# lmmontoya-ai/taboo-brittleness

Measured on AMD Instinct MI355X. Metric: prompts/sec SAE-ablation sweep Gemma-2-9B @L32, higher is better.
Workload: dtype bf16

## Files before the change

taboo_brittleness_amd/csrc/api.h:

```cpp
#pragma once
#include <hip/hip_runtime.h>
#include <stdint.h>

void tb_rmsnorm(const uint16_t* x, const uint16_t* w, uint16_t* y, int M, int D, float eps, hipStream_t st);
void tb_add_rmsnorm2(uint16_t* h, const uint16_t* o, const uint16_t* w_post, const uint16_t* w_next, uint16_t* x,
                     int M, int D, float eps, hipStream_t st);
void tb_embed_rmsnorm(const int32_t* ids, const uint16_t* E, const uint16_t* w, uint16_t* h, uint16_t* x, int M,
                      int D, int V, float scale, float eps, hipStream_t st);
void tb_rope_qkv_cache(const uint16_t* qkv, const int32_t* pos, const int32_t* slot_of_row, const float* cos_t,
                       const float* sin_t, uint16_t* q_out, uint16_t* kc, uint16_t* vc, int M, int Hq, int Hkv,
                       int HD, int S, int max_pos, hipStream_t st);
void tb_rope_qkv_cache_part(const float* part, int ks, const int32_t* pos, const int32_t* slot_of_row,
                            const float* cos_t, const float* sin_t, uint16_t* q_out, uint16_t* kc, uint16_t* vc, int M,
                            int Hq, int Hkv, int HD, int S, int max_pos, hipStream_t st);
void tb_kv_fanout(uint16_t* kc, uint16_t* vc, const int32_t* src_row, const int32_t* slot, const int32_t* pos, int M,
                  int nlayers, int slots, int Hkv, int S, int HD, hipStream_t st);
int tb_attention_lds_bytes(int HD);
int tb_attention_split_rows(int n, bool prefix);
void tb_attention(const uint16_t* q, const uint16_t* kc, const uint16_t* vc, uint16_t* out, const int32_t* pos,
                  const int32_t* slot, int B, int T, int Hq, int Hkv, int HD, int S, float scale, float softcap,
                  int window, hipStream_t st, const uint16_t* pkc = nullptr, const uint16_t* pvc = nullptr,
                  const int32_t* pslot = nullptr, const int32_t* plen = nullptr);
void tb_attention_varlen(const uint16_t* q, const uint16_t* kc, const uint16_t* vc, uint16_t* out, const int32_t* pos,
                         const int32_t* blk, int nblk, int Hq, int Hkv, int HD, int S, float scale, float softcap,
// ... 35 lines not shown
bool tb_gemm4_ok(int M, int N, int K);
int tb_gemm4_set_pipe(int on);
int tb_gemm4_splitk_ks(int M, int N, int K, int tile_rows);
int tb_gemm4_splitk_part(const uint16_t* A, const uint16_t* W, float* ws, int M, int N, int K, int tile_rows, int ks,
                         hipStream_t st);
void tb_add_rmsnorm2_part(uint16_t* h, const float* part, int ks, const uint16_t* w_post, const uint16_t* w_next,
                          uint16_t* x, int M, int D, float eps, hipStream_t st);
void tb_gemm4_splitk(const uint16_t* A, const uint16_t* W, uint16_t* out, float* ws, int M, int N, int K, int ldo,
                     int epi, int tile_rows, int ks, hipStream_t st);
void tb_row_combine(const int64_t* ptr, const float* coef, float* out, int B, int T, int V, hipStream_t st);
bool tb_random_basis_ok(int D);
void tb_random_basis(const uint64_t* seeds, const int32_t* ranks, const int64_t* rows, int n, int D, float* table,
                     hipStream_t st, int qu = 1);
void tb_gemm4(const uint16_t* A, const uint16_t* W, void* C, const float* bias, const float* thr, int M, int N, int K,
              int ldc, int epi, int tile_rows, hipStream_t st, const uint16_t* a2 = nullptr, int k0 = 0);
void tb_gemm_nt(const uint16_t* A, const uint16_t* W, void* C, const float* bias, const float* thr, int M, int N,
                int K, int ldc, int epi, hipStream_t st);
void tb_lowrank_edit(uint16_t* h, uint16_t* x_next, const uint8_t* apply, const int32_t* idx, const int32_t* cnt,
                     int mmax, const void* E, const void* Dm, int table_f32, const float* bias, const float* thr,
                     const float* pre_bias, float alpha, const uint16_t* w_next, float eps, int M, int D,
                     float* coef_out, hipStream_t st, const float* val = nullptr);
void tb_interchange_edit(uint16_t* h, uint16_t* x_next, const uint8_t* apply, const int32_t* idx, const int32_t* cnt,
                         int mmax, const void* E, const void* Dm, int table_f32, const float* bias, const float* thr,
                         const float* pre_bias, float alpha, const uint16_t* w_next, float eps, int M, int D,
                         float* coef_out, const uint16_t* donor, const int32_t* src, int n_donor, float* dcoef_out,
                         hipStream_t st);
void tb_matched_noise_edit(uint16_t* h, uint16_t* x_next, const uint8_t* apply, const int32_t* idx,
                           const int32_t* cnt, int mmax, const void* E, const void* Dm, int table_f32,
                           const float* bias, const float* thr, const float* pre_bias, float alpha,
                           const uint16_t* w_next, float eps, int M, int D, float* coef_out, const float* val,
// ... 68 lines not shown
```

taboo_brittleness_amd/csrc/bindings.cpp:

```cpp
#include <torch/extension.h>
#include <ATen/hip/impl/HIPStreamMasqueradingAsCUDA.h>
#include <c10/core/DeviceGuard.h>

#include <cstdlib>

#include "api.h"

namespace {

hipStream_t cur_stream() { return c10::hip::getCurrentHIPStreamMasqueradingAsCUDA().stream(); }

#define CHECK_DEV(t) TORCH_CHECK((t).is_cuda(), #t " must be a GPU tensor")
#define CHECK_CONTIG(t) TORCH_CHECK((t).is_contiguous(), #t " must be contiguous")
#define CHECK_BF16(t) TORCH_CHECK((t).scalar_type() == at::kBFloat16, #t " must be bfloat16")
#define CHECK_F32(t) TORCH_CHECK((t).scalar_type() == at::kFloat, #t " must be float32")
#define CHECK_I32(t) TORCH_CHECK((t).scalar_type() == at::kInt, #t " must be int32")
#define CHECK_U8(t) TORCH_CHECK((t).scalar_type() == at::kByte || (t).scalar_type() == at::kBool, #t " must be uint8/bool")
#define IN_BF16(t) CHECK_DEV(t); CHECK_CONTIG(t); CHECK_BF16(t)
#define IN_F32(t) CHECK_DEV(t); CHECK_CONTIG(t); CHECK_F32(t)
#define IN_I32(t) CHECK_DEV(t); CHECK_CONTIG(t); CHECK_I32(t)
#define IN_U8(t) CHECK_DEV(t); CHECK_CONTIG(t); CHECK_U8(t)

bool debug_checks() {
  static const bool on = [] {
// ... 589 lines not shown
void gemm4_qkv_rope(torch::Tensor x, torch::Tensor w, torch::Tensor pos, torch::Tensor slot_of_row, torch::Tensor cs,
                    torch::Tensor q_out, torch::Tensor kc, torch::Tensor vc, int64_t Hq, int64_t Hkv,
                    int64_t tile_rows, OptTensor a2) {
  IN_BF16(x); IN_BF16(w);
  int K = x.size(-1), M = pos.numel(), k0 = 0;
  if (given(a2)) l2a_check(x, *a2, w, M, K, k0);
  TORCH_CHECK(x.numel() == (int64_t)M * (k0 ? k0 : K), "gemm4_qkv_rope: x must be [M, K] with M = pos.numel()");
  qkv_l2a_check(pos, slot_of_row, cs, q_out, kc, vc, M, Hq, Hkv, w);
  TORCH_CHECK(w.size(1) == K, "gemm4_qkv_rope: K mismatch");
  TORCH_CHECK(tb_gemm4_ok(M, w.size(0), K), "gemm4_qkv_rope: need K % 64 == 0, K >= 64");
  TORCH_CHECK(tile_rows == 256 || tile_rows == 128, "gemm4_qkv_rope: tile_rows must be 256 or 128");
  c10::DeviceGuard g(x.device());
  tb_gemm4_qkv_rope(cbf(x), cbf(w), pos.data_ptr<int32_t>(), slot_of_row.data_ptr<int32_t>(), cbf(cs),
                    bf(q_out), bf(kc), bf(vc), M, K, Hq, Hkv, kc.size(2), cs.size(0),
                    (int)tile_rows, cur_stream(), k0 ? cbf(*a2) : nullptr, k0);
}

void row_combine(torch::Tensor ptr, torch::Tensor coef, torch::Tensor out) {
  CHECK_DEV(ptr); CHECK_CONTIG(ptr); IN_F32(coef); IN_F32(out);
  TORCH_CHECK(ptr.scalar_type() == at::kLong && ptr.dim() == 2 && coef.sizes() == ptr.sizes(),
              "row_combine: ptr int64 [B, T], coef f32 [B, T]");
  const int B = ptr.size(0), T = ptr.size(1), V = out.size(-1);
  TORCH_CHECK(out.numel() == (int64_t)B * V && V % 4 == 0, "row_combine: out [B, V], V % 4 == 0");
  c10::DeviceGuard g(out.device());
  tb_row_combine(ptr.data_ptr<int64_t>(), coef.data_ptr<float>(), out.data_ptr<float>(), B, T, V, cur_stream());
}

void random_basis(torch::Tensor seeds, torch::Tensor ranks, torch::Tensor rows, torch::Tensor table, int64_t qu) {
  CHECK_DEV(seeds); CHECK_CONTIG(seeds); CHECK_DEV(ranks); CHECK_CONTIG(ranks); CHECK_DEV(rows); CHECK_CONTIG(rows);
  IN_F32(table);
// ... 605 lines not shown
  m.def("gemm_nt", &gemm_nt);
  m.def("gemm4", &gemm4, "A"_a, "W"_a, "C"_a, "bias"_a, "thr"_a, "epi"_a, "tile_rows"_a, a2);
  m.def("gemm4_ok", &gemm4_ok);
  m.def("gemm4_set_pipe", &gemm4_set_pipe);
  m.def("gemm_ring", &gemm_ring, "A"_a, "W"_a, "C"_a, "epi"_a, "bm"_a, "bn"_a, "var"_a, a2);
  m.def("gemm_ring_ok", &gemm_ring_ok);
  m.def("gemm_ring_tiles", &gemm_ring_tiles);
  m.def("gemm_ring_qkv_rope", &gemm_ring_qkv_rope, "x"_a, "w"_a, "pos"_a, "slot_of_row"_a, "cs"_a, "q_out"_a,
        "kc"_a, "vc"_a, "Hq"_a, "Hkv"_a, "bm"_a, "bn"_a, "var"_a, a2);
  m.def("gemm4_splitk", &gemm4_splitk);
  m.def("gemm4_splitk_ks", &gemm4_splitk_ks);
  m.def("gemm4_splitk_part", &gemm4_splitk_part);
  m.def("add_rmsnorm2_part", &add_rmsnorm2_part);
  m.def("gemm4_qkv_rope", &gemm4_qkv_rope, "x"_a, "w"_a, "pos"_a, "slot_of_row"_a, "cs"_a, "q_out"_a, "kc"_a,
        "vc"_a, "Hq"_a, "Hkv"_a, "tile_rows"_a, a2);
  m.def("lora_t", &lora_t);
  m.def("lora_t_chunks", &lora_t_chunks);
  m.def("row_combine", &row_combine);
  m.def("random_basis", &random_basis);
  m.def("lora_t_ok", &lora_t_ok);
  m.def("head_fused", &head_fused);
  m.def("lens_gemm", &lens_gemm);
  m.def("lowrank_edit", &lowrank_edit);
  m.def("latent_affine_edit", &latent_affine_edit);
  m.def("matched_noise_edit", &matched_noise_edit);
  m.def("interchange_edit", &interchange_edit);
  m.def("sae_decode_sparse", &sae_decode_sparse);
  m.def("sae_splice_edit", &sae_splice_edit);
  m.def("flag_compact", &flag_compact);
  m.def("latent_score", &latent_score);
// ... 19 lines not shown
```

taboo_brittleness_amd/csrc/gemm4.hip:

```cpp
#include "common.h"
#include "api.h"
#include <algorithm>
#include <cstdlib>
#include <utility>

namespace {

constexpr int G4_THREADS = 256, G4_BN = 256;
constexpr int G4_GROUP_M = 4;
constexpr int G4_SLACK1 = 4;
constexpr int G4_SLACK2 = 0;
#ifndef G4_CNT
#define G4_CNT 1
#endif

typedef __attribute__((address_space(3))) void g4_lds_t;
typedef uint32_t u32x2 __attribute__((ext_vector_type(2)));
typedef __attribute__((address_space(3))) char g4_lds_char;

template <int N>
__device__ __forceinline__ void g4_vmcnt() {
  static_assert(N >= 0 && N < 64, "vmcnt range");
  asm volatile("s_waitcnt vmcnt(%0)" ::"n"(N) : "memory");
}
// ... 50 lines not shown
  uint16_t* kc;
  uint16_t* vc;
  int Hq, Hkv, S, max_pos;
  const uint16_t* ctab;
  int clo, chi;
  float csat, crc, ccap;
  const int32_t* tgt;
  float* tgt_logit;
  float* part;
  int ksplit, kchunk;
  const uint16_t* a2;
  int k0;
};
constexpr int G4_CTAB_N = 32768;

template <int BM, int EPI, bool L2A = false, bool PIPE = false>
__global__ void __launch_bounds__(G4_THREADS, 1)
gemm4_kernel(const uint16_t* __restrict__ A, const uint16_t* __restrict__ W, void* __restrict__ C,
             const float* __restrict__ bias, const float* __restrict__ thr, int M, int N, int K, int ldc, G4Rope rp) {
#if defined(__HIP_DEVICE_COMPILE__)
  static_assert(BM == 256 || BM == 128 || (BM == 64 && EPI == G4_F32), "tile rows (64: the split-K decode tile)");
  static_assert(!PIPE || (BM == 256 && !L2A && (EPI == G4_BF16 || EPI == G4_LENS || EPI == G4_GEGLU || EPI == G4_ROPE)),
                "cross-tile stream: 256-row tile, one A source, no split-K");
  static_assert(!PIPE || BM == G4_BN, "PIPE stages A with W's row offsets");
  constexpr bool G4C = G4_CNT && BM == 256;
  constexpr int WN = 8, WM = BM / 32;
  constexpr int PIMG = G4_BN * 128, QIMG = BM * 128, STG = PIMG + QIMG;
  constexpr int PI = G4_BN / 32, QI = BM / 32, GL = PI + QI;
  constexpr bool LEPI = EPI == G4_BF16 || EPI == G4_LENS;
  constexpr int RB = EPI == G4_GEGLU ? 128 : 256, ECH = RB / 16, ERPI = 64 / ECH;
  constexpr bool SPARE = LEPI;
  constexpr int EXB = SPARE ? 32768 : 0;
  constexpr int ERR = SPARE ? EXB / (4 * RB) : EPI == G4_GEGLU ? BM / 2 : BM / 4;
  constexpr int ENR = LEPI ? (BM / 2) / ERPI : 1;
  constexpr int CTB = EPI == G4_HEAD ? 4096 : 0;
  static_assert(2 * STG + CTB + EXB <= 160 * 1024, "LDS");
  __shared__ __attribute__((aligned(1024))) char smem[2 * STG + CTB + EXB];

  const int nbn = N / G4_BN, nbm = (M + BM - 1) / BM, nwg = nbn * nbm;
  const int NT = K >> 6, KS = EPI == G4_F32 && rp.ksplit > 1 ? rp.ksplit : 1, KC = KS > 1 ? rp.kchunk : NT;
  const int nwgv = nwg * KS;
#define G4_TILE(v, m0_, n0_)                                                                              \
  do {                                                                                                    \
    const int q_ = nwgv / 8, r_ = nwgv % 8, x_ = (v) % 8;                                                 \
    int b_ = (x_ < r_ ? x_ * (q_ + 1) : r_ * (q_ + 1) + (x_ - r_) * q_) + (v) / 8;                        \
    sk = b_ / nwg;                                                                                        \
    b_ -= sk * nwg;                                                                                       \
    const int pg_ = G4_GROUP_M * nbn, fb_ = (b_ / pg_) * G4_GROUP_M;                                      \
    const int gs_ = min(nbm - fb_, G4_GROUP_M), l_ = b_ % pg_;                                            \
    m0_ = (fb_ + l_ % gs_) * BM;                                                                          \
    n0_ = (l_ / gs_) * G4_BN;                                                                             \
  } while (0)
  int tile = blockIdx.x, m0, n0, sk;
  G4_TILE(tile, m0, n0);

  const int tid = threadIdx.x, lane = tid & 63;
  const int wid = __builtin_amdgcn_readfirstlane(tid >> 6);
  const int wn = wid & 1, wm = wid >> 1;

  const int lchunk = (lane & 7) ^ ((4 * wid + (lane >> 4)) & 7);
  const int wbytes = G4_BN * K * 2;
  const int KA = L2A ? rp.k0 : K, K2 = K - KA, NT0 = KA >> 6;
  uint32_t vp[PI], vq[QI], vq2[L2A ? QI : 1];
#pragma unroll
  for (int i = 0; i < PI; ++i) vp[i] = (uint32_t)((8 * (4 * i + wid) + (lane >> 3)) * K + lchunk * 8) * 2u;
  int mrows, abytes, abytes2 = 0, nt;
  void *wtile, *atile, *atile2 = nullptr;
#define G4_DESC()                                                                                 \
  do {                                                                                            \
    mrows = min(BM, M - m0);                                                                      \
    wtile = (void*)(W + (size_t)n0 * K + sk * KC * 64);                                           \
    atile = (void*)(A + (size_t)m0 * KA + sk * KC * 64);                                          \
    nt = min(KC, NT - sk * KC);                                                                   \
    abytes = mrows * KA * 2;                                                                      \
    int ln_ = __builtin_amdgcn_mbcnt_hi(~0u, __builtin_amdgcn_mbcnt_lo(~0u, 0u));    \
    asm volatile("" : "+v"(ln_));                                                                 \
    const int lc_ = (ln_ & 7) ^ ((4 * wid + (ln_ >> 4)) & 7);                                     \
    _Pragma("unroll") for (int i = 0; i < QI; ++i)                                                \
      vq[i] = (uint32_t)(min(8 * (4 * i + wid) + (ln_ >> 3), mrows - 1) * KA + lc_ * 8) * 2u;     \
    if constexpr (L2A) {                                                                          \
      atile2 = (void*)(rp.a2 + (size_t)m0 * K2);                                                  \
      abytes2 = mrows * K2 * 2;                                                                   \
      _Pragma("unroll") for (int i = 0; i < QI; ++i)                                              \
        vq2[L2A ? i : 0] = (uint32_t)(min(8 * (4 * i + wid) + (ln_ >> 3), mrows - 1) * K2 + lc_ * 8) * 2u; \
    }                                                                                             \
  } while (0)
  G4_DESC();
  int par = 0, m0n = 0, n0n = 0, abytes_n = 0;
// ... 98 lines not shown
  const uint32_t bq0 = lds0 + offq - PIMG + co0, bq1 = lds0 + offq - PIMG + co1;

  if constexpr (EPI == G4_HEAD) {
    if (rp.ctab != nullptr) {
      uint16_t* lt = reinterpret_cast<uint16_t*>(smem + 2 * STG);
      for (int i = tid; i < rp.chi - rp.clo; i += G4_THREADS) lt[i] = rp.ctab[i];
    }
    __syncthreads();
  }
  G4_STAGE(0, 0);
  G4_STAGE(min(1, nt - 1), 1);
  if constexpr (PIPE) G4_NEXT();
  bool first_tile = true;
  for (;;) {
  constexpr bool REREAD = PIPE && EPI == G4_ROPE;
  if (!PIPE || first_tile || REREAD) {
  if (!PIPE || first_tile) {
    if (first_tile || !LEPI) g4_vmcnt<GL>();
    else g4_vmcnt<GL + ENR>();
    g4_bar();
  }
  if (G4C) {
    asm volatile("s_waitcnt lgkmcnt(0)" ::: "memory");
    const uint32_t o_ = par * STG;
    g4_rd(p0[0], bp0 + o_, G4_PK(0));
#pragma unroll
    for (int j = 0; j < WM; ++j) g4_rd(q0[j], bq0 + o_, G4_QK(j));
#pragma unroll
    for (int i = 1; i < WN; ++i) g4_rd(p0[i], bp0 + o_, G4_PK(i));
    if constexpr (PIPE) G4_HOLD_FRAGS();
  } else {
#pragma unroll
    for (int i = 0; i < WN; ++i) p0[i] = frag(par, offp + G4_PROW(i) * 128 + co0);
#pragma unroll
// ... 64 lines not shown
    G4_PERIOD(nt - 1, kt1, true, true, false);
  }
#undef G4_PERIOD
  if (G4C) asm volatile("s_waitcnt lgkmcnt(0)" ::: "memory");
#undef G4_WAIT
#undef G4_POST
#undef G4_MF
#undef G4_MFMA
#undef G4_MFMA0
  if constexpr (!PIPE) {
    g4_vmcnt<0>();
    g4_bar();
  } else if (G4C && !REREAD) {
    G4_HOLD_FRAGS();
  }
  const int em0 = m0, en0 = n0, esk = sk;
  const int next = PIPE ? nwgv : tile + (int)gridDim.x;
  const bool more = PIPE ? has_next : next < nwgv;
  if constexpr (PIPE) {
    tile += (int)gridDim.x;
    m0 = m0n;
    n0 = n0n;
    wtile = wtile_n;
    atile = atile_n;
    abytes = abytes_n;
    par ^= nt & 1;
  }
  if constexpr (LEPI) {
    if (next < nwgv) {
      tile = next;
      G4_TILE(tile, m0, n0);
      G4_DESC();
      G4_STAGE(0, 0);
      if constexpr (SPARE) G4_STAGE(min(1, nt - 1), 1);
    }
    asm volatile("s_nop 15\n\ts_nop 15" ::: "memory");
    const uint32_t reg = (uint32_t)(uintptr_t)((g4_lds_char*)smem) + (SPARE ? 2 * STG + CTB : STG) + wid * ERR * RB;
    uint16_t* obase = reinterpret_cast<uint16_t*>(C) + (size_t)(em0 + wm * (BM / 2)) * ldc;
    const int nrow = min(BM / 2, M - em0 - wm * (BM / 2));
    const auto ors = __builtin_amdgcn_make_buffer_rsrc(obase, 0, nrow > 0 ? nrow * ldc * 2 : 0, 0x00020000);
    int ln = __builtin_amdgcn_mbcnt_hi(~0u, __builtin_amdgcn_mbcnt_lo(~0u, 0u));
    asm volatile("" : "+v"(ln));
    const int oc0 = (EPI == G4_GEGLU ? (en0 >> 1) + wn * 64 : en0 + wn * 128) + (ln % ECH) * 8;
    constexpr int NI = EPI == G4_GEGLU ? WN / 2 : WN, NRA = ECH / ERPI;
    uint32_t wa[NI], ra[NRA];
#pragma unroll
    for (int i = 0; i < NI; ++i) {
// ... 26 lines not shown
          g4_ds_write_b64<jj * 16 * RB>(wa[i], w);
        }
      });
      u32x4 ev[ERR / ERPI];
      g4_unroll<ERR / ERPI>([&](auto kc) {
        constexpr int k = decltype(kc)::value;
        g4_ds_read_b128<(k / NRA) * NRA * ERPI * RB>(ev[k], ra[k % NRA]);
      });
      asm volatile("s_waitcnt lgkmcnt(0)" ::: "memory");
#pragma unroll
      for (int k = 0; k < ERR / ERPI; ++k)
        __builtin_amdgcn_raw_buffer_store_b128(ev[k], ors, ((rnd * ERR + ERPI * k + ln / ECH) * ldc + oc0) * 2, 0, 0);
    });
    if constexpr (!SPARE) {
      g4_bar();
      if (next < nwgv) G4_STAGE(min(1, nt - 1), 1);
    }
  }
  int tj[EPI == G4_HEAD ? WM : 1];
  if constexpr (EPI == G4_HEAD) {
#pragma unroll
    for (int j = 0; j < WM; ++j) {
      const int m = em0 + wm * (BM / 2) + (lane & 15) + j * 16;
      tj[j] = -1;
      if (rp.tgt != nullptr) {
        const int t = rp.tgt[min(m, M - 1)];
        tj[j] = m < M ? t : -1;
      }
    }
  }
  constexpr int RWM = EPI == G4_ROPE ? WM : 1, RWN = EPI == G4_ROPE ? WN / 2 : 1;
// ... 4 lines not shown
    const int mb_ = em0 + wm * (BM / 2) + (lane & 15);
#pragma unroll
    for (int j = 0; j < WM; ++j) {
      const int m = min(mb_ + j * 16, M - 1);
      rpos[j] = mb_ + j * 16 < M ? rp.pos[m] : -1;
      rslt[j] = rp.slot[m];
    }
#pragma unroll
    for (int j = 0; j < RPF; ++j) {
      const int pp = min(max(rpos[j], 0), rp.max_pos - 1);
#pragma unroll
      for (int i = 0; i < WN / 2; ++i)
        rcs[j][i] = *reinterpret_cast<const uint4*>(rp.cs + ((size_t)pp * 128 + wn * 64 + i * 16 + 4 * (lane >> 4)) * 2);
    }
  }
  if (!LEPI && next < nwgv) {
    tile = next;
    G4_TILE(tile, m0, n0);
    G4_DESC();
    G4_STAGE(0, 0);
    G4_STAGE(min(1, nt - 1), 1);
  }
  const uint16_t* ct = reinterpret_cast<const uint16_t*>(smem + 2 * STG);
  if constexpr (!LEPI) asm volatile("s_nop 15\n\ts_nop 15" ::: "memory");

  {
  const int nb = en0 + wn * 128 + 4 * (lane >> 4);
  const int mb = em0 + wm * (BM / 2) + (lane & 15);
  if constexpr (EPI == G4_HEAD || EPI == G4_LENS) {
    float4* part = reinterpret_cast<float4*>(EPI == G4_LENS ? rp.part : reinterpret_cast<float*>(C));
    const int npart = N / 128, pcol = (en0 >> 7) + wn;
    const uint32_t ctb = (uint32_t)(uintptr_t)((g4_lds_char*)smem) + 2 * STG;
    constexpr float L2E = 1.4426950408889634f;
#pragma unroll
// ... 158 lines not shown
  } else {
#pragma unroll
    for (int i = 0; i < WN; ++i)
#pragma unroll
      for (int j = 0; j < WM; ++j) acc[i][j] = (f32x4){0.f, 0.f, 0.f, 0.f};
  }
  }
  g4_vmcnt<0>();
#undef G4_STAGE
#undef G4_STAGE_ONE
#undef G4_HOLD_FRAGS
#undef G4_STAGE_PIPE
#undef G4_NEXT
#undef G4_TILE
#undef G4_DESC
#endif
}

template <int EPI>
__global__ void __launch_bounds__(256) g4_splitk_reduce_kernel(const float* __restrict__ part, uint16_t* __restrict__ out,
                                                               int M, int N, int ks, int ldo) {
  const int nout = EPI == G4_GEGLU ? N / 2 : N;
  const size_t i = (size_t)blockIdx.x * blockDim.x + threadIdx.x;
  const int per_row = nout / 8;
  if (i >= (size_t)M * per_row) return;
  const int m = (int)(i / per_row), c8 = (int)(i % per_row) * 8;
  const size_t plane = (size_t)M * N;
  float o[8];
  if constexpr (EPI == G4_GEGLU) {
    const int blk = c8 >> 6, fi = c8 & 63;
// ... 177 lines not shown
  G4Rope rp{pos, slot_of_row, cs, q_out, kc, vc, Hq, Hkv, S, max_pos};
  if (a2 != nullptr) {
    rp.a2 = a2;
    rp.k0 = k0;
    if (tile_rows == 128) G4_GO2(128, G4_ROPE);
    else G4_GO2(256, G4_ROPE);
    return;
  }
  if (tile_rows == 128) G4_GO(128, G4_ROPE);
  else G4_GOP(G4_ROPE);
#undef G4_GOP
#undef G4_GO
#undef G4_GO2
}

namespace {

__global__ void __launch_bounds__(256) head_merge_kernel(const float4* __restrict__ part, int npart,
                                                         const int32_t* __restrict__ tgt,
                                                         const float* __restrict__ tgt_logit, int32_t* __restrict__ nxt,
                                                         float* __restrict__ nll_self, float* __restrict__ nll_tgt,
                                                         float* __restrict__ lse_out, int V) {
  __shared__ float sm[4], ss[4];
  __shared__ int si[4];
  const int r = blockIdx.x;
  const float4* p = part + (size_t)r * npart;
  float mx = -INFINITY, s = 0.f;
  int bi = 0x7fffffff;
  auto merge = [&](float m2, float s2, int i2) {
    if (m2 > mx) { s = (mx == -INFINITY ? 0.f : s * __expf(mx - m2)) + s2; mx = m2; bi = i2; }
// ... 39 lines not shown
```

taboo_brittleness_amd/isa_check.py:

```python
from __future__ import annotations

import os
import re
import subprocess
import sys
import tempfile
from typing import Dict, List, Set, Tuple

CSRC = os.path.join(os.path.dirname(os.path.abspath(__file__)), "csrc")
HIPCC = os.path.join(os.environ.get("ROCM_PATH", "/opt/rocm"), "bin", "hipcc")

_REG = re.compile(r"\b([va])(?:\[(\d+):(\d+)\]|(\d+)(?!\w))")


def _regs(text: str) -> Set[Tuple[str, int]]:
    out = set()
    for m in _REG.finditer(text):
        kind = m.group(1)
        if m.group(4) is not None:
            out.add((kind, int(m.group(4))))
        else:
            out.update((kind, r) for r in range(int(m.group(2)), int(m.group(3)) + 1))
    return out

# ... 49 lines not shown


def loops(asm: str, variants: bool = False) -> Dict[str, Tuple[List[str], List[str]]]:
    funcs: Dict[str, List[str]] = {}
    cur = None
    for line in asm.split("\n"):
        m = re.match(r"^(_Z\S+):", line)
        if m:
            cur = m.group(1)
            funcs[cur] = []
            continue
        if cur is not None:
            funcs[cur].append(line)
    out = {}
    for name, body in funcs.items():
        m = re.search(r"gemm4_kernelILi(\d+)ELi(\d+)E(?:Lb([01])ELb([01])E)?", name)
        if not m or m.group(1) != "256":
            continue
        blocks, cur_b, labels = [], [], [""]
        for line in body:
            if re.match(r"^\.LBB", line):
                blocks.append(cur_b)
                cur_b = []
                labels.append(line.split(":")[0])
            else:
                s = line.strip()
                if s and not s.startswith((";", ".")):
                    cur_b.append(s.split(";")[0].strip())
        blocks.append(cur_b)
        nmf = [sum("mfma" in x for x in b) for b in blocks]
        pipe = m.group(4) == "1"
        if pipe:
# ... 2 lines not shown
            ti = next((i for i in range(li + 1, len(blocks)) if nmf[i] >= 200), None)
        else:
            li = max(range(len(blocks)), key=lambda i: nmf[i])
            ti = li + 1 if li + 1 < len(blocks) else None
        def _top(blk):
            fm = next((i for i, x in enumerate(blk) if "mfma" in x), len(blk))
            nrd = sum(x.startswith("ds_read_b128") for x in blk[:fm])
            return nrd > 0 and (fm == len(blk) or (pipe and nrd >= 16))

        pi = li - 1
        while pi >= 0 and not _top(blocks[pi]):
            pi -= 1
        pre = [x for b in blocks[max(pi, 0): li] for x in b] if pi >= 0 else []
        key = f"gemm4_kernel<256, {m.group(2)}>"
        if variants:
            key = f"gemm4_kernel<256, {m.group(2)}, {m.group(3) or 0}, {m.group(4) or 0}>"
        elif key in out and (pipe or m.group(3) == "1"):
            continue
        out[key] = (pre, blocks[li])
        tail = []
        if ti is not None:
            last = max([i for i, x in enumerate(blocks[ti]) if "mfma" in x], default=-1)
            for i, x in enumerate(blocks[ti]):
                tail.append(x)
                if i > last and x.startswith("s_waitcnt") and "lgkmcnt(0)" in x:
                    break
        _TAILS[key] = tail
    return out


_TAILS: Dict[str, List[str]] = {}
# ... 48 lines not shown
```

taboo_brittleness_amd/ops/gemm.py:

```python
from __future__ import annotations

from typing import Optional

import torch
import torch.nn.functional as F

from ..runtime import gemm_dispatch as _GD
from . import BF16, _k, _out, add_rmsnorm2, rope_qkv_cache
from . import reference as ref

_WS: dict = {}
_WS_KEEP: list = []


def _workspace(tag: str, n: int, device) -> torch.Tensor:
    key = (tag, device.index, torch.cuda.current_stream(device).stream_id)
    b = _WS.get(key)
    if b is None or b.numel() < n:
        b = torch.empty(max(n, 2 * b.numel() if b is not None else n), dtype=torch.float32, device=device)
        _WS[key] = b
        _WS_KEEP.append(b)
    return b[:n]


def _splitk_part(x, w, tile_rows: int):
    K = x.shape[-1]
    M, N = x.numel() // K, w.shape[0]
    ks = int(_k().gemm4_splitk_ks(M, N, K, tile_rows))
    ws = _workspace("splitk", ks * M * N, x.device)
    return ws, int(_k().gemm4_splitk_part(x, w, ws, tile_rows, ks))


def run_plan(launches, x, w, out, epi: int, a2=None, bias=None, thr=None, rope=None) -> None:
    k = _k()
    M = x.numel() // x.shape[-1]
    pos, slot, cs, kc, vc, Hq, Hkv = rope if rope is not None else (None,) * 7
    for L in launches:
        xa, aa, oa, pa, sa = x, a2, out, pos, slot
        if L.r1 - L.r0 != M:
            xa, aa, oa, pa, sa = (None if t is None else t.reshape(M, -1)[L.r0:L.r1] for t in (x, a2, out, pos, slot))
        if L.family == "g4" and rope is None:
            k.gemm4(xa, w, oa, bias, thr, epi, L.tile, aa)
        elif L.family == "g4":
            k.gemm4_qkv_rope(xa, w, pa, sa, cs, oa, kc, vc, Hq, Hkv, L.tile, aa)
        elif L.family == "ring" and rope is None:
            k.gemm_ring(xa, w, oa, epi, *L.tile, aa)
        elif L.family == "ring":
            k.gemm_ring_qkv_rope(xa, w, pa, sa, cs, oa, kc, vc, Hq, Hkv, *L.tile, aa)
        elif L.family == "splitk" and a2 is None and rope is None:
            N, K = w.shape
            ks = int(k.gemm4_splitk_ks(M, N, K, L.tile))
            k.gemm4_splitk(x, w, out, _workspace("splitk", ks * M * N, x.device), epi, L.tile, ks)
        else:
            raise ValueError(f"no in-tree GEMM launch for {L!r} (epilogue {epi}, {'two' if a2 is not None else 'one'} "
                             "A source)")


def _ring_ok(M: int, N: int, K: int):
    return lambda epi, bm, bn, var: _k().gemm_ring_ok(M, N, K, epi, bm, bn, var)


def tb_gemm(x, w, out, bias, thr, epi: int, choice, a2=None) -> None:
    run_plan(_GD.plan(x.numel() // x.shape[-1], *w.shape, choice=choice), x, w, out, int(epi), a2, bias, thr)
# ... 156 lines not shown
```

taboo_brittleness_amd/runtime/gemm_dispatch.py:

```python
from __future__ import annotations

import bisect
import functools
import json
import os
from typing import Dict, List, NamedTuple, Optional, Tuple, Union

REPO = os.path.dirname(os.path.dirname(os.path.dirname(os.path.abspath(__file__))))
TABLE_DIR = os.path.join(REPO, "configs", "gemm_dispatch")
NUM_CU = 256

Choice = Union[int, str]

_state = {"mode": os.environ.get("TB_GEMM", "tb"), "table": None, "tb_table": None, "table_path": None,
          "loaded": False}


def set_mode(mode: str) -> None:
    assert mode in ("auto", "tb", "blas"), mode
    _state["mode"] = mode


def mode() -> str:
    return _state["mode"]
# ... 67 lines not shown

G128_COST = 0.64


@functools.lru_cache(maxsize=4096)
def split_rows(M: int, N: int) -> int:
    nbn = max(1, N // 256)

    def cost(m1):
        c = -(-nbn * -(-m1 // 256) // NUM_CU) if m1 > 0 else 0
        return c + (G128_COST * -(-nbn * -(-(M - m1) // 128) // NUM_CU) if m1 < M else 0.0)
    cands = [min(256 * k, M) for k in range(-(-M // 256) + 1)]
    return min(cands, key=lambda m1: (cost(m1), -m1))


class Parsed(NamedTuple):
    kind: str
    tile: Union[None, int, Tuple[int, int, int]] = None


class Launch(NamedTuple):
    family: str
    r0: int
    r1: int
    tile: Union[None, int, Tuple[int, int, int]] = None


@functools.lru_cache(maxsize=512, typed=True)
def parse_choice(c) -> Parsed:
    if isinstance(c, Parsed):
        return c
    if isinstance(c, int) and not isinstance(c, bool):
        return Parsed("g", c)
    if isinstance(c, str):
        if c in ("gs", "blas"):
            return Parsed(c)
        head, body = c[:1], c[1:]
        if head in ("g", "k") and body.isdigit():
            return Parsed(head, int(body))
        if head == "r":
            var = {"b": 1, "c": 2}.get(body[-1:], 0)
            bm, _, bn = (body[:-1] if var else body).partition("x")
            if bm.isdigit() and bn.isdigit():
                return Parsed("r", (int(bm), int(bn), var))
    raise ValueError(f"unknown GEMM choice {c!r}")


def is_invariant(choice: Choice) -> bool:
    return isinstance(choice, str) and parse_choice(choice).kind in ("g", "gs", "r")


def ring_tile(choice: Choice) -> Optional[Tuple[int, int, int]]:
    p = parse_choice(choice) if isinstance(choice, str) else None
    return p.tile if p is not None and p.kind == "r" else None


def resolve(M: int, N: int, K: int, epi: int = 0, two_source: bool = False, ring_ok=None) -> Parsed:
    if two_source:
        c = choose(M, N, K, epi)
        p = parse_choice(c) if isinstance(c, str) else None
        if p is not None and p.kind == "r":
            bm, bn, _ = p.tile
            p = Parsed("r", (bm, bn, 1)) if ring_ok(epi if epi in (3, 4) else 0, bm, bn, 1) else None
        return parse_choice(fill_choice(M, N)) if p is None or p.kind in ("blas", "k") else p
# ... 1 lines not shown
        p = parse_choice(choose(M, N, K, 0))
    else:
        p = parse_choice(choose(M, N, K, epi))
    if epi == 3 and p.kind == "blas":
        return parse_choice(fill_choice(M, N))
    if epi == 4 and p.kind == "r" and not ring_ok(4, *p.tile):
        return Parsed("g", 128)
    return p


@functools.lru_cache(maxsize=4096)
def _launches(p: Parsed, M: int, N: int) -> Tuple[Launch, ...]:
    if p.kind == "gs":
        M1 = split_rows(M, N)
        return tuple(Launch("g4", r0, r1, rows) for r0, r1, rows in ((0, M1, 256), (M1, M, 128)) if r1 > r0)
    return (Launch({"g": "g4", "k": "splitk", "r": "ring", "blas": "blas"}[p.kind], 0, M, p.tile),)


def plan(M: int, N: int, K: int, epi: int = 0, two_source: bool = False, ring_ok=None,
         choice: Optional[Choice] = None) -> Tuple[Launch, ...]:
    p = resolve(M, N, K, epi, two_source, ring_ok) if choice is None else parse_choice(choice)
    return _launches(p, M, N)


def describe() -> dict:
    return {"mode": _state["mode"],
            "table": os.path.relpath(_state["table_path"], REPO) if _state["table_path"] else None}
```

Measured before the change: 2749.

## Add stream-K persistent GEMM variant with cross-workgroup partial accumulation

Adds a stream-K mode to the 256-row gemm4 kernel. Each workgroup takes a contiguous range of K-iterations across tiles, writes partial accumulators to a global slab, and signals through flag words. The workgroup that finishes a tile spin-waits on its neighbour's flag and falls back to recomputing the tile if the wait times out. The aim is to cut wave-quantization tail imbalance when the tile count does not divide evenly by the CU count. The cost is extra slab traffic and spin-wait latency. It is only reached when the dispatch table selects the 's256' choice.

```diff
diff --git a/taboo_brittleness_amd/csrc/api.h b/taboo_brittleness_amd/csrc/api.h
--- a/taboo_brittleness_amd/csrc/api.h
+++ b/taboo_brittleness_amd/csrc/api.h
@@ -73,6 +73,17 @@
                      hipStream_t st, int qu = 1);
 void tb_gemm4(const uint16_t* A, const uint16_t* W, void* C, const float* bias, const float* thr, int M, int N, int K,
               int ldc, int epi, int tile_rows, hipStream_t st, const uint16_t* a2 = nullptr, int k0 = 0);
+constexpr size_t TB_G4_SK_SLAB = 256 * 256 * sizeof(float);
+struct TbRopeArgs {
+  const int32_t* pos;
+  const int32_t* slot;
+  const uint16_t* cs;
+  uint16_t *q_out, *kc, *vc;
+  int Hq, Hkv, S, max_pos;
+};
+int tb_gemm4_sk(const uint16_t* A, const uint16_t* W, void* C, int M, int N, int K, int ldc, int epi,
+                const TbRopeArgs* rope, float* slab, size_t slab_bytes, uint32_t* flags, size_t flag_bytes,
+                int grid_override, int wait_budget, hipStream_t st);
 void tb_gemm_nt(const uint16_t* A, const uint16_t* W, void* C, const float* bias, const float* thr, int M, int N,
                 int K, int ldc, int epi, hipStream_t st);
 void tb_lowrank_edit(uint16_t* h, uint16_t* x_next, const uint8_t* apply, const int32_t* idx, const int32_t* cnt,
diff --git a/taboo_brittleness_amd/csrc/bindings.cpp b/taboo_brittleness_amd/csrc/bindings.cpp
--- a/taboo_brittleness_amd/csrc/bindings.cpp
+++ b/taboo_brittleness_amd/csrc/bindings.cpp
@@ -627,6 +627,51 @@
   tb_gemm4_qkv_rope(cbf(x), cbf(w), pos.data_ptr<int32_t>(), slot_of_row.data_ptr<int32_t>(), cbf(cs),
                     bf(q_out), bf(kc), bf(vc), M, K, Hq, Hkv, kc.size(2), cs.size(0),
                     (int)tile_rows, cur_stream(), k0 ? cbf(*a2) : nullptr, k0);
+}
+
+static void sk_ws_check(const torch::Tensor& slab, const torch::Tensor& flags) {
+  CHECK_DEV(slab); CHECK_CONTIG(slab); CHECK_DEV(flags); CHECK_CONTIG(flags);
+  TORCH_CHECK(flags.scalar_type() == at::kInt, "gemm4_sk: flags must be int32");
+  TORCH_CHECK(reinterpret_cast<uintptr_t>(slab.data_ptr()) % 16 == 0, "gemm4_sk: slab must be 16-byte aligned");
+}
+int64_t gemm4_sk(torch::Tensor A, torch::Tensor W, torch::Tensor C, int64_t epi, torch::Tensor slab, torch::Tensor flags,
+                 int64_t grid, int64_t wait_budget) {
+  IN_BF16(A); IN_BF16(W); IN_BF16(C);
+  sk_ws_check(slab, flags);
+  TORCH_CHECK(W.dim() == 2, "gemm4_sk: W must be [N, K]");
+  const int K = A.size(-1), M = A.numel() / K, N = W.size(0);
+  TORCH_CHECK(W.size(1) == K && tb_gemm4_ok(M, N, K), "gemm4_sk: need N % 256 == 0, K % 64 == 0, K >= 64");
+  TORCH_CHECK(epi == 0 || epi == 3, "gemm4_sk: epi must be 0 (bf16) or 3 (GeGLU)");
+  const int64_t ncols = epi == 3 ? N / 2 : N;
+  TORCH_CHECK(C.numel() == (int64_t)M * ncols, "gemm4_sk: C shape");
+  c10::DeviceGuard g(A.device());
+  const int got = tb_gemm4_sk(cbf(A), cbf(W), C.data_ptr(), M, N, K, (int)ncols, (int)epi, nullptr,
+                              reinterpret_cast<float*>(slab.data_ptr()), slab.nbytes(),
+                              reinterpret_cast<uint32_t*>(flags.data_ptr()), flags.nbytes(), (int)grid, (int)wait_budget,
+                              cur_stream());
+  TORCH_CHECK(got > 0, "gemm4_sk: grid must be a multiple of 8 within the CU count, slab >= grid x 256 KB, "
+                       "flags >= grid words");
+  return got;
+}
+int64_t gemm4_sk_qkv_rope(torch::Tensor x, torch::Tensor w, torch::Tensor pos, torch::Tensor slot_of_row,
+                          torch::Tensor cs, torch::Tensor q_out, torch::Tensor kc, torch::Tensor vc, int64_t Hq,
+                          int64_t Hkv, torch::Tensor slab, torch::Tensor flags, int64_t grid, int64_t wait_budget) {
+  IN_BF16(x); IN_BF16(w);
+  sk_ws_check(slab, flags);
+  const int K = x.size(-1), M = pos.numel();
+  TORCH_CHECK(x.numel() == (int64_t)M * K, "gemm4_sk_qkv_rope: x must be [M, K] with M = pos.numel()");
+  qkv_l2a_check(pos, slot_of_row, cs, q_out, kc, vc, M, Hq, Hkv, w);
+  TORCH_CHECK(w.size(1) == K && tb_gemm4_ok(M, w.size(0), K), "gemm4_sk_qkv_rope: need K % 64 == 0, K >= 64");
+  c10::DeviceGuard g(x.device());
+  const TbRopeArgs ra{pos.data_ptr<int32_t>(), slot_of_row.data_ptr<int32_t>(), cbf(cs), bf(q_out), bf(kc), bf(vc),
+                      (int)Hq, (int)Hkv, (int)kc.size(2), (int)cs.size(0)};
+  const int got = tb_gemm4_sk(cbf(x), cbf(w), nullptr, M, (int)w.size(0), K, 0, 4, &ra,
+                              reinterpret_cast<float*>(slab.data_ptr()), slab.nbytes(),
+                              reinterpret_cast<uint32_t*>(flags.data_ptr()), flags.nbytes(), (int)grid, (int)wait_budget,
+                              cur_stream());
+  TORCH_CHECK(got > 0, "gemm4_sk_qkv_rope: grid must be a multiple of 8 within the CU count, slab >= grid x 256 KB, "
+                       "flags >= grid words");
+  return got;
 }
 
 void row_combine(torch::Tensor ptr, torch::Tensor coef, torch::Tensor out) {
@@ -1262,6 +1307,9 @@
   m.def("add_rmsnorm2_part", &add_rmsnorm2_part);
   m.def("gemm4_qkv_rope", &gemm4_qkv_rope, "x"_a, "w"_a, "pos"_a, "slot_of_row"_a, "cs"_a, "q_out"_a, "kc"_a,
         "vc"_a, "Hq"_a, "Hkv"_a, "tile_rows"_a, a2);
+  m.def("gemm4_sk", &gemm4_sk, "A"_a, "W"_a, "C"_a, "epi"_a, "slab"_a, "flags"_a, "grid"_a = 0, "wait_budget"_a = -1);
+  m.def("gemm4_sk_qkv_rope", &gemm4_sk_qkv_rope, "x"_a, "w"_a, "pos"_a, "slot_of_row"_a, "cs"_a, "q_out"_a, "kc"_a,
+        "vc"_a, "Hq"_a, "Hkv"_a, "slab"_a, "flags"_a, "grid"_a = 0, "wait_budget"_a = -1);
   m.def("lora_t", &lora_t);
   m.def("lora_t_chunks", &lora_t_chunks);
   m.def("row_combine", &row_combine);
diff --git a/taboo_brittleness_amd/csrc/gemm4.hip b/taboo_brittleness_amd/csrc/gemm4.hip
--- a/taboo_brittleness_amd/csrc/gemm4.hip
+++ b/taboo_brittleness_amd/csrc/gemm4.hip
@@ -88,7 +88,33 @@
 };
 constexpr int G4_CTAB_N = 32768;
 
-template <int BM, int EPI, bool L2A = false, bool PIPE = false>
+__host__ __device__ inline int g4_sk_snap(int c, int NT) {
+  int t = c / NT, k = (c % NT) & ~1;
+  if (k < 4) k = 0;
+  else if (NT - k < 4) { k = 0; ++t; }
+  return t * NT + k;
+}
+__host__ __device__ inline int g4_sk_cut(int r, int nwg, int NT, int G) {
+  const long long U = (long long)nwg * NT;
+  if (nwg >= G) return g4_sk_snap((int)(r * U / G), NT);
+  int prev = 0;
+  for (int i = 1; i <= r; ++i) {
+    int c = g4_sk_snap((int)(i * U / G), NT);
+    c = c > prev ? c : prev;
+    if (c % NT != 0 && prev % NT != 0 && c / NT == prev / NT) c = (c / NT + 1) * NT;
+    prev = c;
+  }
+  return prev;
+}
+typedef __attribute__((address_space(1))) uint32_t g4_gu32;
+__device__ __forceinline__ void g4_acc_load(f32x4& d, const char* base, uint32_t off) {
+  asm volatile("global_load_dwordx4 %0, %1, %2" : "=a"(d) : "v"(off), "s"(base) : "memory");
+}
+__device__ __forceinline__ void g4_acc_store(char* base, uint32_t off, const f32x4& v) {
+  asm volatile("global_store_dwordx4 %0, %1, %2" ::"v"(off), "a"(v), "s"(base) : "memory");
+}
+
+template <int BM, int EPI, bool L2A = false, bool PIPE = false, bool SK = false>
 __global__ void __launch_bounds__(G4_THREADS, 1)
 gemm4_kernel(const uint16_t* __restrict__ A, const uint16_t* __restrict__ W, void* __restrict__ C,
              const float* __restrict__ bias, const float* __restrict__ thr, int M, int N, int K, int ldc, G4Rope rp) {
@@ -97,6 +123,8 @@
   static_assert(!PIPE || (BM == 256 && !L2A && (EPI == G4_BF16 || EPI == G4_LENS || EPI == G4_GEGLU || EPI == G4_ROPE)),
                 "cross-tile stream: 256-row tile, one A source, no split-K");
   static_assert(!PIPE || BM == G4_BN, "PIPE stages A with W's row offsets");
+  static_assert(!SK || (BM == 256 && !L2A && !PIPE && (EPI == G4_BF16 || EPI == G4_GEGLU || EPI == G4_ROPE)),
+                "stream-K: 256-row tile, one A source, plain loop");
   constexpr bool G4C = G4_CNT && BM == 256;
   constexpr int WN = 8, WM = BM / 32;
   constexpr int PIMG = G4_BN * 128, QIMG = BM * 128, STG = PIMG + QIMG;
@@ -108,8 +136,9 @@
   constexpr int ERR = SPARE ? EXB / (4 * RB) : EPI == G4_GEGLU ? BM / 2 : BM / 4;
   constexpr int ENR = LEPI ? (BM / 2) / ERPI : 1;
   constexpr int CTB = EPI == G4_HEAD ? 4096 : 0;
-  static_assert(2 * STG + CTB + EXB <= 160 * 1024, "LDS");
-  __shared__ __attribute__((aligned(1024))) char smem[2 * STG + CTB + EXB];
+  constexpr int SKB = SK && !SPARE ? 1024 : 0;
+  static_assert(2 * STG + CTB + EXB + SKB <= 160 * 1024, "LDS");
+  __shared__ __attribute__((aligned(1024))) char smem[2 * STG + CTB + EXB + SKB];
 
   const int nbn = N / G4_BN, nbm = (M + BM - 1) / BM, nwg = nbn * nbm;
   const int NT = K >> 6, KS = EPI == G4_F32 && rp.ksplit > 1 ? rp.ksplit : 1, KC = KS > 1 ? rp.kchunk : NT;
@@ -118,6 +147,7 @@
   do {                                                                                                    \
     const int q_ = nwgv / 8, r_ = nwgv % 8, x_ = (v) % 8;                                                 \
     int b_ = (x_ < r_ ? x_ * (q_ + 1) : r_ * (q_ + 1) + (x_ - r_) * q_) + (v) / 8;                        \
+    if constexpr (SK) b_ = (v);                \
     sk = b_ / nwg;                                                                                        \
     b_ -= sk * nwg;                                                                                       \
     const int pg_ = G4_GROUP_M * nbn, fb_ = (b_ / pg_) * G4_GROUP_M;                                      \
@@ -126,6 +156,27 @@
     n0_ = (l_ / gs_) * G4_BN;                                                                             \
   } while (0)
   int tile = blockIdx.x, m0, n0, sk;
+  int sk_p = 0, sk_cnt = 0, sk_prod = 0, sk_w0 = 0, sk_nw = 0, sk_t0 = 0, sk_k0 = 0, sk_t1 = 0, sk_k1 = 0, sk_r = 0;
+  int kb = 0, knt = 0, kind = 0;
+  bool plainw = false;
+#define G4_SK_ENTRY()                                                                    \
+  do {                                                                                   \
+    if (sk_p < sk_prod) { tile = sk_t1; kb = 0; knt = sk_k1; kind = 1; }                 \
+    else if (sk_p - sk_prod < sk_nw) { tile = sk_w0 + sk_p - sk_prod; kb = 0; knt = NT; kind = 0; } \
+    else { tile = sk_t0; kb = sk_k0; knt = NT - sk_k0; kind = 2; }                       \
+  } while (0)
+  if constexpr (SK) {
+    const int G = gridDim.x, b = blockIdx.x;
+    sk_r = (b % 8) * (G / 8) + b / 8;
+    const int c0 = g4_sk_cut(sk_r, nwg, NT, G), c1 = g4_sk_cut(sk_r + 1, nwg, NT, G);
+    if (c1 <= c0) return;
+    sk_t0 = c0 / NT, sk_k0 = c0 % NT, sk_t1 = c1 / NT, sk_k1 = c1 % NT;
+    sk_prod = sk_k1 > 0;
+    sk_w0 = sk_t0 + (sk_k0 > 0);
+    sk_nw = max(sk_t1 - sk_w0, 0);
+    sk_cnt = sk_prod + sk_nw + (sk_k0 > 0);
+    G4_SK_ENTRY();
+  }
   G4_TILE(tile, m0, n0);
 
   const int tid = threadIdx.x, lane = tid & 63;
@@ -143,9 +194,15 @@
 #define G4_DESC()                                                                                 \
   do {                                                                                            \
     mrows = min(BM, M - m0);                                                                      \
-    wtile = (void*)(W + (size_t)n0 * K + sk * KC * 64);                                           \
-    atile = (void*)(A + (size_t)m0 * KA + sk * KC * 64);                                          \
-    nt = min(KC, NT - sk * KC);                                                                   \
+    if constexpr (SK) {                                                                           \
+      wtile = (void*)(W + (size_t)n0 * K + kb * 64);                                              \
+      atile = (void*)(A + (size_t)m0 * KA + kb * 64);                                             \
+      nt = knt;                                                                                   \
+    } else {                                                                                      \
+      wtile = (void*)(W + (size_t)n0 * K + sk * KC * 64);                                         \
+      atile = (void*)(A + (size_t)m0 * KA + sk * KC * 64);                                        \
+      nt = min(KC, NT - sk * KC);                                                                 \
+    }                                                                                             \
     abytes = mrows * KA * 2;                                                                      \
     int ln_ = __builtin_amdgcn_mbcnt_hi(~0u, __builtin_amdgcn_mbcnt_lo(~0u, 0u));    \
     asm volatile("" : "+v"(ln_));                                                                 \
@@ -274,10 +331,49 @@
   bool first_tile = true;
   for (;;) {
   constexpr bool REREAD = PIPE && EPI == G4_ROPE;
+  if constexpr (SK) {
+    if (kind == 2) {
+      volatile __attribute__((address_space(3))) int* okp =
+          (volatile __attribute__((address_space(3))) int*)((g4_lds_char*)smem + 2 * STG + CTB);
+      if (tid == 0) {
+        g4_gu32* fl = (g4_gu32*)(reinterpret_cast<uint32_t*>(rp.tgt_logit) + (sk_r - 1));
+        const uint64_t t0 = __builtin_amdgcn_s_memrealtime();
+        int ok = 0;
+        while (__builtin_amdgcn_s_memrealtime() - t0 < (uint64_t)rp.kchunk) {
+          if (__hip_atomic_load(fl, __ATOMIC_RELAXED, __HIP_MEMORY_SCOPE_AGENT) != 0u) { ok = 1; break; }
+          __builtin_amdgcn_s_sleep(4);
+        }
+        *okp = ok;
+        __builtin_amdgcn_fence(__ATOMIC_ACQUIRE, "agent");
+        asm volatile("s_waitcnt vmcnt(0)" ::: "memory");
+      }
+      __syncthreads();
+      if (__builtin_amdgcn_readfirstlane(*okp) != 0) {
+        const char* sl = reinterpret_cast<const char*>(rp.part) + (size_t)(sk_r - 1) * (WN * WM * G4_THREADS * 16);
+        uint32_t so = tid * 16;
+        asm volatile("" : "+s"(sl), "+v"(so));
+#pragma unroll
+        for (int i = 0; i < WN; ++i)
+#pragma unroll
+          for (int j = 0; j < WM; ++j) g4_acc_load(acc[i][j], sl + (i * WM + j) * (G4_THREADS * 16), so);
+        asm volatile("s_waitcnt vmcnt(0)" ::: "memory");
+      } else {
+        g4_vmcnt<0>();
+        g4_bar();
+        kb = 0;
+        knt = NT;
+        G4_DESC();
+        G4_STAGE(0, 0);
+        G4_STAGE(min(1, nt - 1), 1);
+      }
+      plainw = true;
+    }
+  }
   if (!PIPE || first_tile || REREAD) {
   if (!PIPE || first_tile) {
-    if (first_tile || !LEPI) g4_vmcnt<GL>();
+    if (first_tile || !LEPI || (SK && plainw)) g4_vmcnt<GL>();
     else g4_vmcnt<GL + ENR>();
+    plainw = false;
     g4_bar();
   }
   if (G4C) {
@@ -372,9 +468,52 @@
   } else if (G4C && !REREAD) {
     G4_HOLD_FRAGS();
   }
+  if constexpr (SK) {
+    if (kind == 1) {
+      asm volatile("s_nop 15\n\ts_nop 15" ::: "memory");
+      char* sl = reinterpret_cast<char*>(rp.part) + (size_t)sk_r * (WN * WM * G4_THREADS * 16);
+      uint32_t so = tid * 16;
+      asm volatile("" : "+s"(sl), "+v"(so));
+#pragma unroll
+      for (int i = 0; i < WN; ++i)
+#pragma unroll
+        for (int j = 0; j < WM; ++j) g4_acc_store(sl + (i * WM + j) * (G4_THREADS * 16), so, acc[i][j]);
+      asm volatile("s_waitcnt vmcnt(0)" ::: "memory");
+      __syncthreads();
+      if (tid == 0) {
+        __builtin_amdgcn_fence(__ATOMIC_RELEASE, "agent");
+        asm volatile("s_waitcnt vmcnt(0)" ::: "memory");
+        __hip_atomic_store((g4_gu32*)(reinterpret_cast<uint32_t*>(rp.tgt_logit) + sk_r), 1u, __ATOMIC_RELAXED,
+                           __HIP_MEMORY_SCOPE_AGENT);
+      }
+      if (sk_p + 1 >= sk_cnt) break;
+      ++sk_p;
+      G4_SK_ENTRY();
+      G4_TILE(tile, m0, n0);
+      G4_DESC();
+      G4_STAGE(0, 0);
+      G4_STAGE(min(1, nt - 1), 1);
+#pragma unroll
+      for (int i = 0; i < WN; ++i)
+#pragma unroll
+        for (int j = 0; j < WM; ++j) acc[i][j] = (f32x4){0.f, 0.f, 0.f, 0.f};
+      plainw = true;
+      continue;
+    }
+  }
   const int em0 = m0, en0 = n0, esk = sk;
   const int next = PIPE ? nwgv : tile + (int)gridDim.x;
-  const bool more = PIPE ? has_next : next < nwgv;
+  const bool more = SK ? sk_p + 1 < sk_cnt : PIPE ? has_next : next < nwgv;
+  const bool adv = SK ? more : next < nwgv;
+#define G4_ADV()                          \
+  do {                                    \
+    if constexpr (SK) {                   \
+      ++sk_p;                             \
+      G4_SK_ENTRY();                      \
+    } else tile = next;                   \
+    G4_TILE(tile, m0, n0);                \
+    G4_DESC();                            \
+  } while (0)
   if constexpr (PIPE) {
     tile += (int)gridDim.x;
     m0 = m0n;
@@ -385,10 +524,8 @@
     par ^= nt & 1;
   }
   if constexpr (LEPI) {
-    if (next < nwgv) {
-      tile = next;
-      G4_TILE(tile, m0, n0);
-      G4_DESC();
+    if (adv) {
+      G4_ADV();
       G4_STAGE(0, 0);
       if constexpr (SPARE) G4_STAGE(min(1, nt - 1), 1);
     }
@@ -445,7 +582,7 @@
     });
     if constexpr (!SPARE) {
       g4_bar();
-      if (next < nwgv) G4_STAGE(min(1, nt - 1), 1);
+      if (adv) G4_STAGE(min(1, nt - 1), 1);
     }
   }
   int tj[EPI == G4_HEAD ? WM : 1];
@@ -480,10 +617,8 @@
         rcs[j][i] = *reinterpret_cast<const uint4*>(rp.cs + ((size_t)pp * 128 + wn * 64 + i * 16 + 4 * (lane >> 4)) * 2);
     }
   }
-  if (!LEPI && next < nwgv) {
-    tile = next;
-    G4_TILE(tile, m0, n0);
-    G4_DESC();
+  if (!LEPI && adv) {
+    G4_ADV();
     G4_STAGE(0, 0);
     G4_STAGE(min(1, nt - 1), 1);
   }
@@ -672,6 +807,8 @@
 #undef G4_NEXT
 #undef G4_TILE
 #undef G4_DESC
+#undef G4_ADV
+#undef G4_SK_ENTRY
 #endif
 }
 
@@ -879,6 +1016,35 @@
 #undef G4_GO2
 }
 
+int tb_gemm4_sk(const uint16_t* A, const uint16_t* W, void* C, int M, int N, int K, int ldc, int epi,
+                const TbRopeArgs* rope, float* slab, size_t slab_bytes, uint32_t* flags, size_t flag_bytes,
+                int grid_override, int wait_budget, hipStream_t st) {
+  if (!tb_gemm4_ok(M, N, K) || slab == nullptr || flags == nullptr) return 0;
+  if (!(epi == G4_BF16 || epi == G4_GEGLU || (epi == G4_ROPE && rope != nullptr))) return 0;
+  const int cap = g4_grid(1 << 30);
+  const int grid = grid_override > 0 ? grid_override : cap;
+  if (grid % 8 != 0 || grid > cap) return 0;
+  if (slab_bytes < (size_t)grid * TB_G4_SK_SLAB || flag_bytes < (size_t)grid * sizeof(uint32_t)) return 0;
+  G4Rope rp{};
+  if (epi == G4_ROPE)
+    rp = G4Rope{rope->pos, rope->slot, rope->cs, rope->q_out, rope->kc, rope->vc, rope->Hq, rope->Hkv, rope->S,
+                rope->max_pos};
+  rp.part = slab;
+  rp.tgt_logit = reinterpret_cast<float*>(flags);
+  rp.kchunk = (wait_budget < 0 ? 200 : std::min(wait_budget, 10000000)) * 100;
+  (void)hipMemsetAsync(flags, 0, (size_t)grid * sizeof(uint32_t), st);
+  const float* bias = nullptr;
+  const float* thr = nullptr;
+#define G4_GOS(E_)                                                                                              \
+  hipLaunchKernelGGL((gemm4_kernel<256, E_, false, false, true>), dim3(grid), dim3(G4_THREADS), 0, st, A, W, C,  \
+                     bias, thr, M, N, K, ldc, rp)
+  if (epi == G4_BF16) G4_GOS(G4_BF16);
+  else if (epi == G4_GEGLU) G4_GOS(G4_GEGLU);
+  else G4_GOS(G4_ROPE);
+#undef G4_GOS
+  return grid;
+}
+
 namespace {
 
 __global__ void __launch_bounds__(256) head_merge_kernel(const float4* __restrict__ part, int npart,
diff --git a/taboo_brittleness_amd/isa_check.py b/taboo_brittleness_amd/isa_check.py
--- a/taboo_brittleness_amd/isa_check.py
+++ b/taboo_brittleness_amd/isa_check.py
@@ -87,8 +87,11 @@
             funcs[cur].append(line)
     out = {}
     for name, body in funcs.items():
-        m = re.search(r"gemm4_kernelILi(\d+)ELi(\d+)E(?:Lb([01])ELb([01])E)?", name)
+        m = re.search(r"gemm4_kernelILi(\d+)ELi(\d+)E(?:Lb([01])ELb([01])E)?(?:Lb([01])E)?", name)
         if not m or m.group(1) != "256":
+            continue
+        sk = m.group(5) == "1"
+        if sk and not variants:
             continue
         blocks, cur_b, labels = [], [], [""]
         for line in body:
@@ -121,7 +124,7 @@
         pre = [x for b in blocks[max(pi, 0): li] for x in b] if pi >= 0 else []
         key = f"gemm4_kernel<256, {m.group(2)}>"
         if variants:
-            key = f"gemm4_kernel<256, {m.group(2)}, {m.group(3) or 0}, {m.group(4) or 0}>"
+            key = f"gemm4_kernel<256, {m.group(2)}, {m.group(3) or 0}, {m.group(4) or 0}{', 1' if sk else ''}>"
         elif key in out and (pipe or m.group(3) == "1"):
             continue
         out[key] = (pre, blocks[li])
diff --git a/taboo_brittleness_amd/ops/gemm.py b/taboo_brittleness_amd/ops/gemm.py
--- a/taboo_brittleness_amd/ops/gemm.py
+++ b/taboo_brittleness_amd/ops/gemm.py
@@ -21,6 +21,15 @@
         _WS[key] = b
         _WS_KEEP.append(b)
     return b[:n]
+
+
+SK_SLAB_BYTES = 256 * 256 * 4
+_SK_MAX_GRID = 256
+
+
+def _sk_workspace(device):
+    ws = _workspace("sk", _SK_MAX_GRID + _SK_MAX_GRID * SK_SLAB_BYTES // 4, device)
+    return ws[_SK_MAX_GRID:], ws[:_SK_MAX_GRID].view(torch.int32)
 
 
 def _splitk_part(x, w, tile_rows: int):
@@ -47,6 +56,12 @@
             k.gemm_ring(xa, w, oa, epi, *L.tile, aa)
         elif L.family == "ring":
             k.gemm_ring_qkv_rope(xa, w, pa, sa, cs, oa, kc, vc, Hq, Hkv, *L.tile, aa)
+        elif L.family == "sk" and a2 is None and epi in (0, 3, 4) and L.tile == 256:
+            slab, flags = _sk_workspace(x.device)
+            if rope is None:
+                k.gemm4_sk(xa, w, oa, epi, slab, flags)
+            else:
+                k.gemm4_sk_qkv_rope(xa, w, pa, sa, cs, oa, kc, vc, Hq, Hkv, slab, flags)
         elif L.family == "splitk" and a2 is None and rope is None:
             N, K = w.shape
             ks = int(k.gemm4_splitk_ks(M, N, K, L.tile))
diff --git a/taboo_brittleness_amd/runtime/gemm_dispatch.py b/taboo_brittleness_amd/runtime/gemm_dispatch.py
--- a/taboo_brittleness_amd/runtime/gemm_dispatch.py
+++ b/taboo_brittleness_amd/runtime/gemm_dispatch.py
@@ -105,6 +105,40 @@
     return min(cands, key=lambda m1: (cost(m1), -m1))
 
 
+SK_MIN_SEG = 4
+
+
+def _sk_snap(c: int, NT: int) -> int:
+    t, k = divmod(c, NT)
+    k &= ~1
+    if k < SK_MIN_SEG:
+        k = 0
+    elif NT - k < SK_MIN_SEG:
+        t, k = t + 1, 0
+    return t * NT + k
+
+
+def sk_cuts(nwg: int, NT: int, G: int) -> List[int]:
+    U, cuts = nwg * NT, [0]
+    for r in range(1, G + 1):
+        c = max(_sk_snap(r * U // G, NT), cuts[-1])
+        if c % NT and cuts[-1] % NT and c // NT == cuts[-1] // NT:
+            c = (c // NT + 1) * NT
+        cuts.append(c)
+    return cuts
+
+
+def sk_entries(nwg: int, NT: int, G: int, r: int) -> List[Tuple[int, int, int, str]]:
+    cuts = sk_cuts(nwg, NT, G)
+    c0, c1 = cuts[r], cuts[r + 1]
+    if c1 <= c0:
+        return []
+    (t0, k0), (t1, k1) = divmod(c0, NT), divmod(c1, NT)
+    out = [(t1, 0, k1, "head")] if k1 else []
+    out += [(t, 0, NT, "whole") for t in range(t0 + (k0 > 0), t1)]
+    return out + ([(t0, k0, NT - k0, "tail")] if k0 else [])
+
+
 class Parsed(NamedTuple):
     kind: str
     tile: Union[None, int, Tuple[int, int, int]] = None
@@ -127,7 +161,7 @@
         if c in ("gs", "blas"):
             return Parsed(c)
         head, body = c[:1], c[1:]
-        if head in ("g", "k") and body.isdigit():
+        if head in ("g", "k") and body.isdigit() or c == "s256":
             return Parsed(head, int(body))
         if head == "r":
             var = {"b": 1, "c": 2}.get(body[-1:], 0)
@@ -138,7 +172,7 @@
 
 
 def is_invariant(choice: Choice) -> bool:
-    return isinstance(choice, str) and parse_choice(choice).kind in ("g", "gs", "r")
+    return isinstance(choice, str) and parse_choice(choice).kind in ("g", "gs", "r", "s")
 
 
 def ring_tile(choice: Choice) -> Optional[Tuple[int, int, int]]:
@@ -170,7 +204,7 @@
     if p.kind == "gs":
         M1 = split_rows(M, N)
         return tuple(Launch("g4", r0, r1, rows) for r0, r1, rows in ((0, M1, 256), (M1, M, 128)) if r1 > r0)
-    return (Launch({"g": "g4", "k": "splitk", "r": "ring", "blas": "blas"}[p.kind], 0, M, p.tile),)
+    return (Launch({"g": "g4", "k": "splitk", "s": "sk", "r": "ring", "blas": "blas"}[p.kind], 0, M, p.tile),)
 
 
 def plan(M: int, N: int, K: int, epi: int = 0, two_source: bool = False, ring_ok=None,
```

New measurement: 2710. 0.986x the previous value.
